# Aakash1312/Fluid-Simulation

Measured on AMD Instinct MI355X. Metric: simulated substeps/sec, higher is better.
Workload: dtype f64

## Files before the change

fluid-simulation_amd/_lib.py:

```python
import ctypes as C
import os

_HERE = os.path.dirname(os.path.abspath(__file__))
_SO = os.path.join(_HERE, "libfluid_hip.so")
if not os.path.exists(_SO):
    raise ImportError(
        f"{_SO} is missing: build it with `make -C {_HERE}` (hipcc --offload-arch=gfx950). "
        "This package has no CPU path.")
lib = C.CDLL(_SO)


class FluidError(RuntimeError):
    def __init__(self, code, msg):
        super().__init__(f"libfluid_hip error {code}: {msg}")
        self.code = code


class Params(C.Structure):
    _fields_ = [("n", C.c_int32), ("device", C.c_int32), ("dx", C.c_double), ("rho", C.c_double),
                ("gravity", C.c_double * 3), ("max_dt", C.c_double), ("outer_tol", C.c_double),
                ("update_frac", C.c_double), ("cg_tol", C.c_double), ("cg_max_iters", C.c_int32),
                ("max_outer_passes", C.c_int32), ("precision", C.c_int32), ("preconditioner", C.c_int32),
                ("flip_blend", C.c_double), ("solve_start", C.c_int32), ("mg_precision", C.c_int32),
                ("dist_solve", C.c_int32), ("pad_", C.c_int32)]
# ... 120 lines not shown
    ("fluid_download_particles", C.c_int, [_P, _P, _P]),
    ("fluid_num_particles", C.c_int64, [_P]),
    ("fluid_set_dt", C.c_int, [_P, C.c_double]),
    ("fluid_get_dt", C.c_int, [_P, C.POINTER(C.c_double)]),
    ("fluid_scene_water_cube_drop", C.c_int64, [C.c_int32, C.c_int32, C.c_uint64, _P]),
    ("fluid_scene_uniform_scatter", C.c_int64, [C.POINTER(C.c_int32), C.POINTER(C.c_int32), C.c_float, C.c_uint32, C.c_int32, _P]),
    ("fluid_step", C.c_int, [_P, C.POINTER(StepStats)]),
    ("fluid_p2g", C.c_int, [_P]),
    ("fluid_flags_index", C.c_int, [_P]),
    ("fluid_rhs_div", C.c_int, [_P, C.c_int]),
    ("fluid_solve", C.c_int, [_P]),
    ("fluid_vel_update", C.c_int, [_P]),
    ("fluid_pressure_pass", C.c_int, [_P, C.POINTER(C.c_double)]),
    ("fluid_flip_advect", C.c_int, [_P]),
    ("fluid_get_stats", C.c_int, [_P, C.POINTER(StepStats)]),
    ("fluid_download_field", C.c_int, [_P, C.c_int, _P, C.c_size_t]),
    ("fluid_upload_field", C.c_int, [_P, C.c_int, _P, C.c_size_t]),
    ("fluid_stencil_apply", C.c_int, [_P, C.c_int, C.c_int, C.POINTER(C.c_float)]),
    ("fluid_extrapolate", C.c_int, [_P, C.POINTER(C.c_int32)]),
    ("fluid_resample", C.c_int, [_P, C.c_int32, C.POINTER(C.c_int64)]),
    ("fluid_get_droplets", C.c_int, [_P, C.POINTER(C.c_int32), _P, C.c_int32]),
    ("fluid_add_particles", C.c_int, [_P, C.c_int64, _P, _P]),
    ("fluid_set_source", C.c_int, [_P, C.c_int32, C.POINTER(Source)]),
    ("fluid_set_sink", C.c_int, [_P, C.c_int32, C.POINTER(C.c_int32), C.POINTER(C.c_int32)]),
    ("fluid_get_source_stats", C.c_int, [_P, C.POINTER(C.c_int64), C.POINTER(C.c_int64), C.POINTER(C.c_int64), C.POINTER(C.c_int64)]),
    ("fluid_dist_set_source", C.c_int, [_P, C.c_int32, C.POINTER(Source)]),
    ("fluid_dist_set_sink", C.c_int, [_P, C.c_int32, C.POINTER(C.c_int32), C.POINTER(C.c_int32)]),
    ("fluid_dist_get_source_stats", C.c_int, [_P, C.POINTER(C.c_int64), C.POINTER(C.c_int64), C.POINTER(C.c_int64), C.POINTER(C.c_int64)]),
    ("fluid_dist_add_particles", C.c_int, [_P, C.c_int64, _P, _P, _P]),
    ("fluid_stencil_apply_hbm", C.c_int, [_P, C.c_int, C.c_int, C.c_int64, C.POINTER(C.c_int32), C.POINTER(C.c_float)]),
# ... 104 lines not shown
```

fluid-simulation_amd/csrc/fluid_api.hip:

```cpp
#include "sim.h"
#include <algorithm>

using namespace fl;

static thread_local std::string g_err;
int fluid_fail(int code, const std::string& msg)
{
    g_err = msg;
    return code;
}
#define fail fluid_fail

Box fl::clip_dilate(const Box& b, int d, const Grid& g)
{
    Box r;
    r.x0 = b.x0 - d < 0 ? 0 : b.x0 - d;
    r.y0 = b.y0 - d < 0 ? 0 : b.y0 - d;
    r.z0 = b.z0 - d < 0 ? 0 : b.z0 - d;
    r.x1 = b.x1 + d > g.nx - 1 ? g.nx - 1 : b.x1 + d;
    r.y1 = b.y1 + d > g.ny - 1 ? g.ny - 1 : b.y1 + d;
    r.z1 = b.z1 + d > g.nz - 1 ? g.nz - 1 : b.z1 + d;
    return r;
}

// ... 37 lines not shown
    }
}


static void free_particles(fluid_sim* s)
{
    for (Particles* p : {&s->pa, &s->pb}) {
        hipFree(p->px); hipFree(p->py); hipFree(p->pz); hipFree(p->vx); hipFree(p->vy); hipFree(p->vz); hipFree(p->pid);
        *p = Particles{};
    }
    hipFree(s->key); hipFree(s->slot); hipFree(s->order); hipFree(s->order2); hipFree(s->spid); hipFree(s->stage_pos); hipFree(s->stage_vel);
    s->order2 = nullptr; s->spid = nullptr; hipFree(s->pw);
    s->pw = nullptr;
    s->key = s->slot = s->order = nullptr;
    s->binned = false;
    s->stage_pos = s->stage_vel = nullptr;
    s->cap = 0;
}

int fl::alloc_particles(fluid_sim* s, long n)
{
    if (n <= s->cap) return FLUID_OK;
    n = (n + 1) & ~1L;
    free_particles(s);
    for (Particles* p : {&s->pa, &s->pb}) {
        HIPCHK(dalloc(&p->px, n)); HIPCHK(dalloc(&p->py, n)); HIPCHK(dalloc(&p->pz, n));
        HIPCHK(dalloc(&p->vx, n)); HIPCHK(dalloc(&p->vy, n)); HIPCHK(dalloc(&p->vz, n));
        HIPCHK(dalloc(&p->pid, n));
    }
    HIPCHK(dalloc(&s->key, n)); HIPCHK(dalloc(&s->slot, n)); HIPCHK(dalloc(&s->order, n)); HIPCHK(dalloc(&s->order2, n)); HIPCHK(dalloc(&s->spid, n));
    HIPCHK(dalloc(&s->stage_pos, 3 * n)); HIPCHK(dalloc(&s->stage_vel, 3 * n));
    HIPCHK(dalloc(&s->pw, 9 * n));
    HIPCHK(hipDeviceSynchronize());
    s->cap = n;
    return FLUID_OK;
}

int fl::grow_particles(fluid_sim* s, long need)
{
    if (need <= s->cap) return FLUID_OK;
    HIPCHK(hipStreamSynchronize(s->st));
    const long keep = s->p_off + s->np;
    Particles old = s->pa;
    s->pa = Particles{};
    const long ncap = ((need + need / 2) + 1) & ~1L;
    Particles nw{};
    HIPCHK(dalloc(&nw.px, ncap)); HIPCHK(dalloc(&nw.py, ncap)); HIPCHK(dalloc(&nw.pz, ncap));
    HIPCHK(dalloc(&nw.vx, ncap)); HIPCHK(dalloc(&nw.vy, ncap)); HIPCHK(dalloc(&nw.vz, ncap));
    HIPCHK(dalloc(&nw.pid, ncap));
    if (keep > 0) {
        HIPCHK(hipMemcpy(nw.px, old.px, keep * 8, hipMemcpyDeviceToDevice)); HIPCHK(hipMemcpy(nw.py, old.py, keep * 8, hipMemcpyDeviceToDevice));
        HIPCHK(hipMemcpy(nw.pz, old.pz, keep * 8, hipMemcpyDeviceToDevice)); HIPCHK(hipMemcpy(nw.vx, old.vx, keep * 8, hipMemcpyDeviceToDevice));
        HIPCHK(hipMemcpy(nw.vy, old.vy, keep * 8, hipMemcpyDeviceToDevice)); HIPCHK(hipMemcpy(nw.vz, old.vz, keep * 8, hipMemcpyDeviceToDevice));
        HIPCHK(hipMemcpy(nw.pid, old.pid, keep * 4, hipMemcpyDeviceToDevice));
    }
    hipFree(old.px); hipFree(old.py); hipFree(old.pz); hipFree(old.vx); hipFree(old.vy); hipFree(old.vz); hipFree(old.pid);
// ... 46 lines not shown
    if (s->st) hipStreamSynchronize(s->st);
    if (s->ds) dist_destroy(s);
    prof_resolve(s);
    free_particles(s);
    sources_free(s);
    output_free(s);
    render_free(s);
    mesh_free(s);
    sdf_free(s);
    void* ptrs[] = {s->solid, s->flags, s->container, s->rhs, s->diver, s->diver2, s->u, s->v, s->w, s->ub, s->vb, s->wb, s->dcx, s->dcy,
                    s->dcz, s->pressure, s->p_guess, s->p_guess2, s->p_q, s->indices, s->scan_sums, s->ipart, s->R, s->S[0], s->Q, s->X, s->mg_slab, s->mg_part, s->cntL, s->part_bb, s->part_rr,
                    s->part_rz[0], s->part_rz[1], s->part_pq, s->part_err, s->cell_count, s->cell_start, s->ss,
                    s->pcx, s->pcy, s->pcz, s->p2g_part, s->p2g_items, s->p2g_crowd, s->tl_flags, s->tl_mg, s->tl_sq, s->d_small, s->row_flags, s->row_pos, s->row_list, s->drop_n, s->drop_cells, s->drop_ctr, s->gal_slab};
    for (void* p : ptrs) if (p) hipFree(p);
    for (int i = 0; i < 2; ++i) if (s->ev_poll[i]) hipEventDestroy(s->ev_poll[i]);
    if (s->h_ss) hipHostFree(s->h_ss);
    if (s->h_small) hipHostFree(s->h_small);
    if (s->st) hipStreamDestroy(s->st);
    delete s;
    return FLUID_OK;
}

int fluid_create(const fluid_params_t* p, fluid_sim_t** out)
{
    if (!p || !out) return fail(FLUID_ERR_ARG, "null argument");
    Grid g;
    g.N = p->n;
    g.lo = -(p->n / 2);
    g.hi = g.lo + p->n - 1;
    g.nx = g.ny = g.nz = p->n;
// ... 23 lines not shown
    s->prm = *p;
    s->g = g;
    s->ncell = g.cells();
    s->dt = p->max_dt;
    s->mg_fp32 = p->mg_precision == FLUID_MG_FP32;
    s->warm = p->solve_start == FLUID_START_WARM;
    if (const char* e = getenv("FLUID_MG_CSWEEPS")) s->mg_csweeps = atoi(e);
    if (const char* e = getenv("FLUID_TILE_LISTS")) s->lists_force = atoi(e) != 0;
    if (const char* e = getenv("FLUID_P2G_FORM")) s->p2g_force = !strcmp(e, "rows") ? 1 : (!strcmp(e, "tiles") ? 2 : (!strcmp(e, "crowd") ? 3 : 0));
    if (const char* e = getenv("FLUID_MG_GALERKIN")) s->gal_mode = atoi(e);
    if (const char* e = getenv("FLUID_DROPLETS")) s->drops_on = atoi(e) != 0;
    if (const char* e = getenv("FLUID_ROW_SWEEPS")) s->row_sweeps = atoi(e) != 0;
    if (const char* e = getenv("FLUID_DROPLETS_MIN")) s->drop_min = atoi(e);
    if (const char* e = getenv("FLUID_ADVECT_BIN")) s->advect_bin = atoi(e) != 0;
    if (const char* e = getenv("FLUID_SOLVE_TAIL")) s->solve_tail = atoi(e) != 0;
    *out = nullptr;
    auto bail = [&](int rc) { fluid_destroy(s); return rc; };
#define A(expr) do { hipError_t e_ = (expr); if (e_ != hipSuccess) return bail(fail(FLUID_ERR_HIP, std::string(#expr) + ": " + hipGetErrorString(e_))); } while (0)
    A(hipStreamCreateWithFlags(&s->st, hipStreamNonBlocking));
    const size_t n = s->ncell;
    A(dalloc(&s->solid, n)); A(dalloc(&s->flags, n));
    A(dalloc(&s->container, n)); A(dalloc(&s->rhs, n)); A(dalloc(&s->diver, n)); A(dalloc(&s->diver2, n));
    A(dalloc(&s->u, n)); A(dalloc(&s->v, n)); A(dalloc(&s->w, n));
    A(dalloc(&s->ub, n)); A(dalloc(&s->vb, n)); A(dalloc(&s->wb, n));
    A(dalloc(&s->dcx, n)); A(dalloc(&s->dcy, n)); A(dalloc(&s->dcz, n));
    A(dalloc(&s->pressure, n));
    if (s->warm) {
        A(dalloc(&s->p_guess, n)); A(dalloc(&s->p_guess2, n));
        if (hipMemset(s->p_guess, 0, n * sizeof(double)) != hipSuccess || hipMemset(s->p_guess2, 0, n * sizeof(double)) != hipSuccess) return bail(FLUID_ERR_HIP);
        if (const char* e = getenv("FLUID_EXTRAPOLATE")) s->extrapolate = atoi(e) != 0;
// ... 8 lines not shown
    A(dalloc((char**)&s->R, ln * se)); A(dalloc((char**)&s->S[0], 2 * ln * se + 256));
    s->S[1] = (char*)s->S[0] + ln * se;
    A(dalloc((char**)&s->Q, ln * se)); A(dalloc((char**)&s->X, ln * se)); A(dalloc(&s->cntL, ln + 64));
    A(dalloc(&s->mg_part, ln / 256 + 64));
    A(dalloc(&s->part_bb, (size_t)MAX_PARTIALS)); A(dalloc(&s->part_rr, (size_t)MAX_PARTIALS));
    A(dalloc(&s->part_rz[0], (size_t)MAX_PARTIALS)); A(dalloc(&s->part_rz[1], (size_t)MAX_PARTIALS));
    A(dalloc(&s->part_pq, (size_t)MAX_PARTIALS)); A(dalloc(&s->part_err, (size_t)2 * MAX_PARTIALS));
    static_assert(sizeof(StepState) <= STATE_PS_OFF, "PcgState overlaps StepState");
    A(dalloc((char**)&s->ss, STATE_PS_OFF + sizeof(PcgState)));
    s->ps = (PcgState*)((char*)s->ss + STATE_PS_OFF);
    A(dalloc(&s->cell_count, n + 4)); A(dalloc(&s->cell_start, n + 4));
    A(dalloc(&s->d_small, (size_t)32));
    A(hipHostMalloc((void**)&s->h_small, 32 * sizeof(int)));
    A(hipEventCreateWithFlags(&s->ev_poll[0], hipEventDisableTiming));
    A(hipEventCreateWithFlags(&s->ev_poll[1], hipEventDisableTiming));
    A(hipHostMalloc((void**)&s->h_ss, STATE_PS_OFF + 2 * sizeof(PcgState)));
    s->h_ps = (PcgState*)((char*)s->h_ss + STATE_PS_OFF);
#undef A
    std::vector<uint8_t> sol(n, 0);
    const int N = p->n;
    for (int x = 0; x < g.nx; ++x)
        for (int y = 0; y < g.ny; ++y)
            for (int z = 0; z < g.nz; ++z) {
                const int X = x + g.ox, Y = y + g.oy, Z = z + g.oz;
                if (X < 2 || X > N - 3 || Y < 2 || Y > N - 3 || Z < 2 || Z > N - 3) sol[g.idx(x, y, z)] = 1;
            }
    hipError_t e = hipMemcpy(s->solid, sol.data(), n, hipMemcpyHostToDevice);
    if (e == hipSuccess) e = hipMemcpy(s->flags, sol.data(), n, hipMemcpyHostToDevice);
    if (e == hipSuccess) e = hipDeviceSynchronize();
    if (e != hipSuccess) return bail(fail(FLUID_ERR_HIP, std::string("solid upload: ") + hipGetErrorString(e)));
// ... 24 lines not shown
    HIPCHK(hipStreamSynchronize(s->st));
    HIPCHK(hipMemcpy(s->solid, sol.data(), s->ncell, hipMemcpyHostToDevice));
    HIPCHK(hipMemcpy(s->flags, sol.data(), s->ncell, hipMemcpyHostToDevice));
    s->have_p2g = s->have_flags = false;
    s->flags_valid = false;
    s->have_guess = false;
    return FLUID_OK;
}

int fluid_upload_particles(fluid_sim_t* s, int64_t n, const double* pos, const double* vel)
{
    if (!s || n < 0 || (n > 0 && !pos)) return fail(FLUID_ERR_ARG, "bad particle arguments");
    if (s->dist) return fail(FLUID_ERR_STATE, "decomposed run: use fluid_upload_particles_ids (global ids must be unique across ranks)");
    if (n > 0x7fffffffL) return fail(FLUID_ERR_ARG, "too many particles");
    HIPCHK(hipSetDevice(s->prm.device));
    int rc = alloc_particles(s, (long)n);
    if (rc) return rc;
    s->np = (long)n;
    s->p_off = 0;
    if (n > 0) {
        HIPCHK(hipMemcpyAsync(s->stage_pos, pos, 3 * n * sizeof(double), hipMemcpyHostToDevice, s->st));
        if (vel) HIPCHK(hipMemcpyAsync(s->stage_vel, vel, 3 * n * sizeof(double), hipMemcpyHostToDevice, s->st));
        launch_unpack_particles(s->st, s->np, s->stage_pos, vel ? s->stage_vel : nullptr, s->pa);
        HIPCHK(hipGetLastError());
        HIPCHK(hipStreamSynchronize(s->st));
    }
    s->sorted = s->have_p2g = s->have_flags = false;
    s->have_guess = false;
    s->sort_hint = false;
    s->binned = false;
    s->vel_ok = false;
    return FLUID_OK;
}

int fluid_download_particles(fluid_sim_t* s, double* pos, double* vel)
{
    if (!s || !pos || !vel) return fail(FLUID_ERR_ARG, "null argument");
    if (s->dist) return fail(FLUID_ERR_STATE, "decomposed run: use fluid_download_particles_ids");
    if (s->np == 0) return FLUID_OK;
    HIPCHK(hipSetDevice(s->prm.device));
    launch_pack_particles(s->st, s->np, s->pa.shifted(s->p_off), s->stage_pos, s->stage_vel);
    HIPCHK(hipGetLastError());
    HIPCHK(hipMemcpyAsync(pos, s->stage_pos, 3 * s->np * sizeof(double), hipMemcpyDeviceToHost, s->st));
    HIPCHK(hipMemcpyAsync(vel, s->stage_vel, 3 * s->np * sizeof(double), hipMemcpyDeviceToHost, s->st));
    HIPCHK(hipStreamSynchronize(s->st));
    return FLUID_OK;
}

int64_t fluid_num_particles(fluid_sim_t* s) { return s ? s->np : -1; }
int fluid_set_dt(fluid_sim_t* s, double dt)
{
    if (!s || !(dt > 0)) return fail(FLUID_ERR_ARG, "dt must be > 0");
    s->dt = dt;
    return FLUID_OK;
}
int fluid_get_dt(fluid_sim_t* s, double* dt)
// ... 31 lines not shown
                        cnt++;
                    }
                }
    return cnt;
}

}

int fl::read_ss(fluid_sim* s)
{
    HIPCHK(hipMemcpyAsync(s->h_ss, s->ss, sizeof(StepState), hipMemcpyDeviceToHost, s->st));
    HIPCHK(hipStreamSynchronize(s->st));
    return FLUID_OK;
}

int fl::clear_dirty(fluid_sim* s)
{
    if (box_empty(s->dirty)) return FLUID_OK;
    const ZeroList z = {{s->container, s->rhs, s->diver, s->diver2}, {s->u, s->v, s->w, s->ub, s->vb, s->wb, s->pressure}};
    launch_zero_fields(s->st, z, s->g, s->dirty, !s->dist && s->row_sweeps);
    HIPCHK(hipGetLastError());
    s->dirty = Box{0, 0, 0, -1, -1, -1};
    return FLUID_OK;
}

int fl::sort_pass(fluid_sim* s, int ax0, int ax1, int* h_tail)
{
    const Grid g = s->g;
    const long ncell = (long)s->ncell, n2 = g.sx();
    const long c0 = (long)ax0 * n2, c1 = (long)(ax1 + 1) * n2;
    launch_zero_step_state(s->st, s->ss, g.N);
    HIPCHK(hipMemsetAsync(s->cell_count + c0, 0, (c1 - c0) * sizeof(int), s->st));
    HIPCHK(hipMemsetAsync(s->cell_count + ncell, 0, 4 * sizeof(int), s->st));
    launch_bin_count(s->st, g, s->np, s->pa.shifted(s->p_off), s->key, s->slot, s->cell_count, s->ipart, s->ss);
    launch_exclusive_scan(s->st, s->cell_count + c0, s->cell_start + c0, c1 - c0, s->scan_sums, s->cell_start + c1);
    launch_sort_tail(s->st, s->cell_count, s->cell_start, c1, ncell);
    launch_bin_scatter(s->st, s->np, s->key, s->slot, s->cell_start, s->pa.shifted(s->p_off).pid, s->order, s->spid);
    launch_bin_rank(s->st, s->np, 0, s->key, s->cell_start, s->order, s->spid, s->order2);
    HIPCHK(hipGetLastError());
    if (h_tail) HIPCHK(hipMemcpyAsync(h_tail, s->cell_start + ncell, 3 * sizeof(int), hipMemcpyDeviceToHost, s->st));
    return read_ss(s);
}

static int sort_binned(fluid_sim* s)
{
    const Grid g = s->g;
    const long ncell = (long)s->ncell, n2 = g.sx();
    const long c0 = (long)s->bin_x0 * n2, c1 = (long)(s->bin_x1 + 1) * n2;
    launch_zero_step_state(s->st, s->ss, g.N);
    launch_exclusive_scan(s->st, s->cell_count + c0, s->cell_start + c0, c1 - c0, s->scan_sums, s->cell_start + c1);
    launch_sort_tail(s->st, s->cell_count, s->cell_start, c1, ncell);
    launch_bin_scatter(s->st, s->np, s->key, s->slot, s->cell_start, s->pa.shifted(s->p_off).pid, s->order, s->spid);
    launch_bin_rank(s->st, s->np, 0, s->key, s->cell_start, s->order, s->spid, s->order2);
    HIPCHK(hipGetLastError());
    StepState& h = *s->h_ss;
    for (int a = 0; a < 3; ++a) h.bbox_min[a] = s->bin_min[a], h.bbox_max[a] = s->bin_max[a];
    h.n_out = s->bin_n_out;
    h.max_cell = s->bin_max_cell;
    return FLUID_OK;
}

static int phase_sort(fluid_sim* s)
{
    const Grid g = s->g;
    int tok = prof_begin(s, FLUID_PROF_SORT, (double)s->np);
    int ax0 = 0, ax1 = g.nx - 1;
    const bool guess = s->sort_hint && !box_empty(s->Pb);
    if (guess) {
        ax0 = std::max(0, s->Pb.x0 - 3);
        ax1 = std::min(g.nx - 1, s->Pb.x1 + 3);
    }
    const bool binned = s->binned && guess && ax0 == s->bin_x0 && ax1 == s->bin_x1 && s->np > 0;
    s->binned = false;
    const auto missed = [&](const int* bmin, const int* bmax) {
        return guess && bmax[0] >= 0 && (bmin[0] < std::min(ax0 + 2, s->Pb.x0) || bmax[0] > std::max(ax1 - 2, s->Pb.x1));
    };
    int rc;
    if (binned && !missed(s->bin_min, s->bin_max)) {
        if ((rc = sort_binned(s))) return rc;
    } else {
        rc = binned ? FLUID_OK : sort_pass(s, ax0, ax1);
        if (rc) return rc;
        if (binned || missed(s->h_ss->bbox_min, s->h_ss->bbox_max)) {
            if ((rc = sort_pass(s, 0, g.nx - 1))) return rc;
        }
    }
    s->sort_hint = true;
    s->n_out = s->h_ss->n_out;
    s->max_cell = s->h_ss->max_cell;
    const StepState& h = *s->h_ss;
    if (h.bbox_max[0] < 0) {
        s->Pb = Box{0, 0, 0, -1, -1, -1};
    } else {
        s->Pb = Box{h.bbox_min[0], h.bbox_min[1], h.bbox_min[2], h.bbox_max[0], h.bbox_max[1], h.bbox_max[2]};
    }
    if (!box_empty(s->Pb)) {
        s->Rb = clip_dilate(s->Pb, 1, g);
        s->Sb = clip_dilate(s->Pb, 2, g);
    } else {
        s->Rb = s->Sb = s->Pb;
    }
    launch_reorder(s->st, s->np, s->order2, s->pa.shifted(s->p_off), s->pb, s->pw, s->cap);
    HIPCHK(hipGetLastError());
    std::swap(s->pa, s->pb);
    s->p_off = 0;
    prof_end(s, FLUID_PROF_SORT, tok);
    s->sorted = true;
    return FLUID_OK;
}

int fl::run_p2g(fluid_sim* s, const Box& box)
{
    const long ref_cells = s->p2g_ref_cells > 0 ? s->p2g_ref_cells : s->Rb.cells();
    const bool airy = s->last_num_active > 0 && (double)s->last_num_active < 0.3 * (double)ref_cells;
    const bool huge = (size_t)12 * sizeof(double) * (size_t)box.cells() > ((size_t)16 << 30);
    const bool piled = s->max_cell > P2G_PILED || airy;
    if (s->p2g_force ? s->p2g_force == 2 : huge) {
        s->stats.paths |= FLUID_PATH_P2G_TILES;
        launch_p2g_tiles(s->st, s->g, box, s->pa, s->pw, s->cap, s->cell_start, s->flags, s->container, s->u, s->v, s->w, s->ub, s->vb, s->wb);
        return FLUID_OK;
// ... 467 lines not shown
                    HIPCHK(hipStreamSynchronize(s->st));
                    hipFree(s->row_flags); hipFree(s->row_pos); hipFree(s->row_list);
                    s->row_flags = s->row_pos = s->row_list = nullptr;
                    const size_t cap = nr + nr / 4 + 1024;
                    HIPCHK(hipMalloc((void**)&s->row_flags, cap * sizeof(int)));
                    HIPCHK(hipMalloc((void**)&s->row_pos, cap * sizeof(int)));
                    HIPCHK(hipMalloc((void**)&s->row_list, cap * sizeof(int)));
                    s->row_cap = cap;
                }
                launch_row_list(s->st, s->L, s->cntL, s->row_flags, s->row_pos, s->row_list, s->scan_sums, &s->ss->n_rows);
            }
            built = true;
        }
        HIPCHK(hipGetLastError());
    }
    int rc = read_ss(s);
    if (rc) return rc;
    s->stats.num_active = s->h_ss->num_active;
    s->last_num_active = s->stats.num_active;
    s->lists_on = false;
    s->lists_hint = false;
    if (!box_empty(s->Rb)) {
        const bool airy = (double)s->stats.num_active < 0.45 * (double)s->L.cells() && s->L.cells() > (size_t)1500000;
        s->lists_hint = airy;
        s->n_tl_mg = s->h_ss->n_tl_mg; s->n_tl_sq = s->h_ss->n_tl_sq; s->n_rows = s->h_ss->n_rows;
        s->n_drop = drops ? std::min(s->h_ss->n_drop, DROP_CAP) : 0;
        if (drops) s->drop_last = s->n_drop;
        if (s->n_drop > 0) s->stats.paths |= FLUID_PATH_DROPLETS;
        s->lists_on = built && s->n_tl_mg > 0 && s->n_tl_sq > 0 && (s->lists_force == 1 || airy);
        if (s->lists_on) s->stats.paths |= FLUID_PATH_TILE_LISTS;
        const size_t lb = (s->L.cells() + 2 * (size_t)s->L.Lz) * solver_elem(s);
        HIPCHK(zero_search(s, lb));
        HIPCHK(hipGetLastError());
        if (use_mg(s)) {
            int rc2 = mg_setup(s);
            if (rc2) return rc2;
        }
    }
    s->have_flags = true;
    return FLUID_OK;
}

static int phase_rhs_div(fluid_sim* s, int which, const PcgState* gate)
{
    if (!s->have_flags) return fail(FLUID_ERR_STATE, "rhs_div before flags_index");
    if (box_empty(s->Rb)) return FLUID_OK;
    const double dt = s->dt;
    launch_rhs_div(s->st, s->g, s->Rb, s->flags, s->u, s->v, s->w, s->rhs, which ? s->diver2 : s->diver, s->prm.dx,
                   s->prm.gravity[0] * dt, s->prm.gravity[1] * dt, s->prm.gravity[2] * dt, !s->dist && s->row_sweeps, gate);
    HIPCHK(hipGetLastError());
    return FLUID_OK;
// ... 143 lines not shown
    prof_end(s, FLUID_PROF_G2P, tok);
    const bool bin = s->advect_bin && !s->dist && s->np > 0 && s->sorted && s->sort_hint && !box_empty(s->Pb);
    s->binned = false;
    if (bin) {
        const Grid g = s->g;
        s->bin_x0 = std::max(0, s->Pb.x0 - 3);
        s->bin_x1 = std::min(g.nx - 1, s->Pb.x1 + 3);
        const long n2 = g.sx(), c0 = (long)s->bin_x0 * n2, c1 = (long)(s->bin_x1 + 1) * n2;
        HIPCHK(hipMemsetAsync(s->cell_count + c0, 0, (c1 - c0) * sizeof(int), s->st));
        HIPCHK(hipMemsetAsync(s->cell_count + s->ncell, 0, 4 * sizeof(int), s->st));
        launch_advect_bin(s->st, g, s->np, s->pa.shifted(s->p_off), s->flags, s->prm.max_dt, s->prm.dx, s->ss, s->key, s->slot, s->cell_count, s->ipart);
    } else {
        launch_advect(s->st, s->g, s->np, s->pa.shifted(s->p_off), s->flags, s->prm.max_dt, s->prm.dx, s->ss);
    }
    HIPCHK(hipGetLastError());
    int rc = read_ss(s);
    if (rc) return rc;
    if (bin) {
        const StepState& h = *s->h_ss;
        for (int a = 0; a < 3; ++a) s->bin_min[a] = h.bbox_min[a], s->bin_max[a] = h.bbox_max[a];
        s->bin_n_out = h.n_out;
        s->bin_max_cell = h.max_cell;
        s->binned = true;
    }
    s->dt = s->h_ss->dt;
    double ms;
    memcpy(&ms, &s->h_ss->max_speed_bits, sizeof(double));
    s->stats.max_speed = ms;
    s->stats.dt_out = s->dt;
    s->sorted = false;
    s->have_p2g = false;
    s->vel_ok = true;
    return FLUID_OK;
}

extern "C" {

#define PHASE_GUARD(s)                                                                                        \
// ... 85 lines not shown
    HIPCHK(hipStreamSynchronize(s->st));
    if (n_parked) *n_parked = s->h_small[0];
    s->sorted = s->have_p2g = s->have_flags = false;
    s->sort_hint = false;
    s->binned = false;
    return FLUID_OK;
}

int fluid_get_stats(fluid_sim_t* s, fluid_step_stats_t* st)
{
    if (!s || !st) return fail(FLUID_ERR_ARG, "null argument");
    *st = s->stats;
    return FLUID_OK;
}


int fluid_step(fluid_sim_t* s, fluid_step_stats_t* stats)
{
    if (!s) return fail(FLUID_ERR_ARG, "null handle");
    int rc;
    if ((rc = output_auto_check(s))) return rc;
    if (s->dist) return dist_step(s, stats);
    if ((rc = phase_p2g(s))) return rc;
    if ((rc = phase_flags(s))) return rc;
    double error = NAN;
    do {
        if ((rc = phase_pressure_pass(s, &error))) return rc;
        if (s->prm.max_outer_passes > 0 && s->stats.outer_passes >= s->prm.max_outer_passes) break;
    } while (error > s->prm.outer_tol);
    if ((rc = phase_flip_advect(s))) return rc;
// ... 245 lines not shown
```

fluid-simulation_amd/csrc/fluid_dist.hip:

```cpp
#include "sim.h"
#include "dist_kernels.h"

using namespace fl;
#define fail fluid_fail
int cuts_from_hist(int n, const int64_t* hist, int P, int32_t* cuts);

#define COMMCHK(expr)                                                                              \
    do {                                                                                           \
        if ((expr) != 0) return fail(FLUID_ERR_HIP, std::string("comm callback failed: ") + #expr); \
    } while (0)

namespace {

constexpr int HALO_W = 4;

struct IBox {
    int lo[3], hi[3];
};
inline bool ib_empty(const IBox& b) { return b.hi[0] <= b.lo[0] || b.hi[1] <= b.lo[1] || b.hi[2] <= b.lo[2]; }
inline IBox ib_isect(const IBox& a, const IBox& b)
{
    IBox r;
    for (int k = 0; k < 3; ++k) { r.lo[k] = std::max(a.lo[k], b.lo[k]); r.hi[k] = std::min(a.hi[k], b.hi[k]); }
    if (ib_empty(r)) for (int k = 0; k < 3; ++k) { r.lo[k] = a.lo[k]; r.hi[k] = a.lo[k]; }
// ... 1688 lines not shown
    for (int a = 0; a < 3; ++a) {
        if (origin) origin[a] = o[a];
        if (dims) dims[a] = n[a];
        if (own_lo) own_lo[a] = s->ds ? s->ds->ob.lo[a] : 0;
        if (own_hi) own_hi[a] = s->ds ? s->ds->ob.hi[a] : g.N;
    }
    return FLUID_OK;
}

int fluid_upload_particles_ids(fluid_sim_t* s, int64_t n, const double* pos, const double* vel, const uint32_t* ids)
{
    if (!s || n < 0 || (n > 0 && (!pos || !ids))) return fail(FLUID_ERR_ARG, "bad particle arguments");
    HIPCHK(hipSetDevice(s->prm.device));
    long slack = 1L << 16;
    if (const char* e = getenv("FLUID_DIST_SLACK")) slack = std::max(16L, atol(e));
    int rc = alloc_particles(s, 2 * (long)n + slack);
    if (rc) return rc;
    DistState* d = s->ds;
    if (d && !d->mig_s) {
        d->mig_cap = (long)n / 2 + slack;
        HIPCHK(hipMalloc((void**)&d->mig_s, (size_t)d->mig_cap * 56));
        HIPCHK(hipMalloc((void**)&d->mig_r, (size_t)d->mig_cap * 56));
    }
    s->np = (long)n;
    s->p_off = 0;
    if (n > 0) {
        uint32_t* dids = (uint32_t*)s->order;
        HIPCHK(hipMemcpyAsync(s->stage_pos, pos, 3 * n * sizeof(double), hipMemcpyHostToDevice, s->st));
        if (vel) HIPCHK(hipMemcpyAsync(s->stage_vel, vel, 3 * n * sizeof(double), hipMemcpyHostToDevice, s->st));
        HIPCHK(hipMemcpyAsync(dids, ids, n * sizeof(uint32_t), hipMemcpyHostToDevice, s->st));
// ... 7 lines not shown
    if (d) {
        s->vel_ok = false;
        for (int64_t i = 0; i < n; ++i) d->max_id = std::max(d->max_id, (long long)ids[i]);
    }
    return FLUID_OK;
}

int64_t fluid_download_particles_ids(fluid_sim_t* s, double* pos, double* vel, uint32_t* ids)
{
    if (!s) return -1;
    if (hipSetDevice(s->prm.device) != hipSuccess) return -1;
    int* cursor = s->d_small;
    if (hipMemsetAsync(cursor, 0, sizeof(int), s->st) != hipSuccess) return -1;
    const bool fetch = pos && vel && ids;
    uint32_t* dids = (uint32_t*)s->order;
    launch_pack_live(s->st, s->np, s->pa.shifted(s->p_off), fetch ? s->stage_pos : nullptr, s->stage_vel, dids, cursor);
    int live = 0;
    if (hipMemcpyAsync(s->h_small, cursor, sizeof(int), hipMemcpyDeviceToHost, s->st) != hipSuccess) return -1;
    if (hipStreamSynchronize(s->st) != hipSuccess) return -1;
    live = s->h_small[0];
    if (!fetch || live == 0) return live;
    if (hipMemcpyAsync(pos, s->stage_pos, 3 * (size_t)live * sizeof(double), hipMemcpyDeviceToHost, s->st) != hipSuccess) return -1;
    if (hipMemcpyAsync(vel, s->stage_vel, 3 * (size_t)live * sizeof(double), hipMemcpyDeviceToHost, s->st) != hipSuccess) return -1;
    if (hipMemcpyAsync(ids, dids, (size_t)live * sizeof(uint32_t), hipMemcpyDeviceToHost, s->st) != hipSuccess) return -1;
    if (hipStreamSynchronize(s->st) != hipSuccess) return -1;
    return live;
}

int fluid_partition_blocks(int32_t n, int64_t np, const double* pos, const int32_t dims[3], int32_t* cuts_x, int32_t* cuts_y, int32_t* cuts_z)
{
    if (n < 8 || !dims || !cuts_x || !cuts_y || !cuts_z || (np > 0 && !pos)) return fail(FLUID_ERR_ARG, "bad argument");
// ... 125 lines not shown
```

fluid-simulation_amd/csrc/fluid_sdf.hip:

```cpp
#include "sim.h"

using namespace fl;
#define fail fluid_fail

constexpr size_t SDF_REC = FLUID_SDF_LEAF_BYTES;
struct SdfMeta {
    int wide = 0;
    int attr = 0;
    int n_leaves = 0;
    float bg = 0, R = 0, w = 0;
};
struct SdfState {
    long cell_cap = 0, part_cap = 0, leaf_cap = 0;
    int *cnt = nullptr, *start = nullptr, *cell_sums = nullptr;
    int* place = nullptr;
    double* spos = nullptr;
    float* tv = nullptr;
    float* tv2 = nullptr;
    bool filtered = false;
    int* ssrc = nullptr;
    uint32_t* tid = nullptr;
    float* tvel = nullptr;
    bool attr = false;
    float* tmin = nullptr;
// ... 111 lines not shown
    const float mn = std::fmax(0.0f, R - w);
    g.min2 = mn * mn;
    f->any = false;
    f->tv = nullptr, f->flags = nullptr;
    f->filt = filt, f->dilate = 4;
    f->attr = false, f->dist2 = false;
    f->tm = nullptr, f->tid = nullptr, f->tvel = nullptr, f->tmin = nullptr;
    return FLUID_OK;
}

int fl::sdf_front(fluid_sim* s, SdfFront* f)
{
    SdfState* o = s->sdf;
    SdfGeom& g = f->g;
    int rc;
    const Particles live = s->pa.shifted(s->p_off);
    int* box = o->h_small;
    if (s->np > 0) {
        launch_sdf_bbox(s->st, s->np, live, g.lo, g.hi, o->d_small, s->dist);
        HIPCHK(hipGetLastError());
        HIPCHK(hipMemcpyAsync(o->h_small, o->d_small, 6 * sizeof(int), hipMemcpyDeviceToHost, s->st));
        HIPCHK(hipStreamSynchronize(s->st));
    }
    if (s->np > 0 && box[3] >= box[0]) {
        for (int a = 0; a < 3; ++a)
            if (box[a] < g.lo || box[3 + a] > g.hi || box[3 + a] < box[a]) return fail(FLUID_ERR_HIP, "level set: particle box out of range");
        g.bx0 = box[0], g.by0 = box[1], g.bz0 = box[2];
        g.bnx = box[3] - box[0] + 1, g.bny = box[4] - box[1] + 1, g.bnz = box[5] - box[2] + 1;
        for (int a = 0; a < 3; ++a) {
            const int c0 = std::max(box[a] - f->dilate, g.lo), c1 = std::min(box[3 + a] + f->dilate, g.hi);
            g.l0[a] = (c0 - g.L0) >> 3;
// ... 214 lines not shown
```

fluid-simulation_amd/csrc/fluid_sources.hip:

```cpp
#include "sim.h"
#include <algorithm>

using namespace fl;
#define fail fluid_fail

const char* const fl::SRC_SINGLE = "these entry points are single-GPU only (they renumber the pids): a decomposed handle uses fluid_dist_set_source, fluid_dist_set_sink, fluid_dist_get_source_stats, fluid_dist_add_particles";
const char* const fl::SRC_DIST = "not a decomposed handle: a fluid_create handle uses the one-GPU entry points (fluid_set_source, fluid_set_sink, fluid_get_source_stats, fluid_add_particles)";

static bool index_box(const fluid_sim* s, const int32_t lo[3], const int32_t hi[3], Box& b)
{
    const int N = s->g.N;
    for (int a = 0; a < 3; ++a)
        if (lo[a] < 0 || hi[a] > N - 1 || lo[a] > hi[a]) return false;
    b = Box{lo[0], lo[1], lo[2], hi[0], hi[1], hi[2]};
    return true;
}

static int ensure_sums(fluid_sim* s)
{
    if (s->src_sums) return FLUID_OK;
    HIPCHK(hipMalloc((void**)&s->src_sums, ((size_t)INT32_MAX / 2048 + 16) * sizeof(int)));
    return FLUID_OK;
}

// ... 134 lines not shown
    std::swap(s->pa, s->pb);
    s->p_off = 0;
    s->np = n - r;
    *removed = r;
    return FLUID_OK;
}

int fl::sources_apply(fluid_sim* s)
{
    s->src_emit_last = s->src_rm_last = 0;
    bool any = false;
    for (int i = 0; i < FLUID_MAX_SINKS; ++i) any = any || s->sink_on[i];
    for (const auto& q : s->src) any = any || q.on;
    if (!any) return FLUID_OK;
    s->binned = false;
    const long t = s->n_steps;
    const int N = s->g.N;
    const OwnBox all{{0, 0, 0}, {N, N, N}, {0, 0, 0}, {0, 0, 0}};
    long removed = 0, emitted = 0;
    int rc = apply_sinks(s, &removed);
    if (rc) return rc;
    for (auto& q : s->src) {
        if (!q.on || t % q.src.every != 0) continue;
        const SrcDue u = source_due(s, q, t, all);
        long m = 0, mo = 0;
        if ((rc = source_count(s, u)) || (rc = source_plan(s, u, &m, &mo))) return rc;
        if (m == 0) continue;
        if ((rc = source_room(s, m))) return rc;
        const Particles p = s->pa.shifted(s->p_off + s->np);
        source_emit(s, u, p, (uint32_t)s->np);
// ... 62 lines not shown
    if (emitted_total) *emitted_total = s->src_emit_total;
    if (removed_total) *removed_total = s->src_rm_total;
    return FLUID_OK;
}

extern "C" {

int fluid_add_particles(fluid_sim_t* s, int64_t n, const double* pos, const double* vel)
{
    if (int rc = snap_guard(s, SRC_SINGLE)) return rc;
    if (n < 0 || (n > 0 && !pos)) return fail(FLUID_ERR_ARG, "bad particle arguments");
    if (!vel && !s->vel_ok) return fail(FLUID_ERR_STATE, "add_particles with vel == NULL needs the grid velocities of a completed step");
    if (s->np + (long)n > (long)INT32_MAX) return fail(FLUID_ERR_STATE, "more than INT32_MAX particles");
    if (n == 0) return FLUID_OK;
    HIPCHK(hipSetDevice(s->prm.device));
    int rc = grow_particles(s, s->p_off + s->np + (long)n);
    if (rc) return rc;
    HIPCHK(hipMemcpyAsync(s->stage_pos, pos, 3 * n * sizeof(double), hipMemcpyHostToDevice, s->st));
    if (vel) HIPCHK(hipMemcpyAsync(s->stage_vel, vel, 3 * n * sizeof(double), hipMemcpyHostToDevice, s->st));
    const Particles p = s->pa.shifted(s->p_off + s->np);
    launch_src_append(s->st, (long)n, s->stage_pos, vel ? s->stage_vel : nullptr, p, (uint32_t)s->np);
    if (!vel) launch_interp_from_grid(s->st, s->g, (long)n, p, s->u, s->v, s->w);
    HIPCHK(hipGetLastError());
    HIPCHK(hipStreamSynchronize(s->st));
    s->np += (long)n;
    s->sorted = s->have_p2g = s->have_flags = false;
    s->sort_hint = false;
    s->binned = false;
    return FLUID_OK;
}
// ... 21 lines not shown
```

fluid-simulation_amd/csrc/sim.h:

```cpp
#pragma once
#include "common.h"
#include "../../include/fluid_hip.h"

#include <cmath>
#include <cstdio>
#include <cstdlib>
#include <cstring>
#include <string>
#include <utility>
#include <vector>

int fluid_fail(int code, const std::string& msg);
#define HIPCHK(expr)                                                                                              \
    do {                                                                                                          \
        hipError_t e_ = (expr);                                                                                   \
        if (e_ != hipSuccess)                                                                                     \
            return fluid_fail(FLUID_ERR_HIP, std::string(#expr) + ": " + hipGetErrorString(e_) + " @" + std::to_string(__LINE__)); \
    } while (0)
#include "snap_ring.h"

using namespace fl;

struct ProfClass {
    long launches = 0, sampled = 0;
// ... 86 lines not shown
    long p2g_ref_cells = 0;
    long last_num_active = 0;
    StepState* ss = nullptr;
    StepState* h_ss = nullptr;
    Box Pb{0, 0, 0, -1, -1, -1}, Rb{0, 0, 0, -1, -1, -1}, Sb{0, 0, 0, -1, -1, -1};
    Box dirty{0, 0, 0, -1, -1, -1};
    int flag_x0 = 0, flag_x1 = -1;
    bool flags_valid = false;
    bool sorted = false, have_p2g = false, have_flags = false;
    long n_out = 0;
    bool sort_hint = false;
    bool advect_bin = true;
    bool binned = false;
    int bin_x0 = 0, bin_x1 = -1;
    int bin_min[3] = {0, 0, 0}, bin_max[3] = {-1, -1, -1}, bin_n_out = 0, bin_max_cell = 0;
    bool solve_tail = true;
    bool tail_ran = false;
    double dt = 0.1;
    fluid_step_stats_t stats{};
    static constexpr int MG_MAXL = 8;
    int mg_nl = 0, mg_tail = 0;
    long mg_last_iters_k[3] = {0, 0, 0};
    int pass_class() const { return stats.outer_passes < 2 ? stats.outer_passes : 2; }
    int mg_csweeps = 3;
    MLevel mgl[MG_MAXL];
    uint8_t *mg_typ[MG_MAXL] = {}, *mg_cnt[MG_MAXL] = {};
    int gal_mode = 1;
    int gal_it[2] = {-1, -1};
    int gal_since_probe = 0;
    bool gal_eligible = false;
// ... 61 lines not shown
inline int grid_leaves(const Grid& g) { return ((g.hi & ~7) - (g.lo & ~7)) / 8 + 1; }
inline int snap_guard(const fluid_sim* s, const char* why, bool want_dist = false)
{
    if (!s) return fluid_fail(FLUID_ERR_ARG, "null handle");
    return s->dist != want_dist ? fluid_fail(FLUID_ERR_STATE, why) : FLUID_OK;
}
constexpr const char* ATTR_SINGLE = "these surface attribute calls are single-GPU only: a decomposed handle gives a rank record with squared distances (fluid_dist_sdf_snapshot_attr) and the records merge on the host (fluid_sdf_attr_grids_merge)";
inline size_t solver_elem(const fluid_sim* s) { return s->prm.precision == FLUID_PRECISION_FP32 ? 4 : 8; }
inline bool use_mg(const fluid_sim* s) { return s->prm.preconditioner == FLUID_PRECOND_MG && s->prm.precision == FLUID_PRECISION_FP64; }

int prof_begin(fluid_sim* s, int k, double cells);
void prof_end(fluid_sim* s, int k, int tok);
int alloc_particles(fluid_sim* s, long n);
int grow_particles(fluid_sim* s, long need);
int read_ss(fluid_sim* s);
int sort_pass(fluid_sim* s, int ax0, int ax1, int* h_tail = nullptr);
int clear_dirty(fluid_sim* s);
int run_p2g(fluid_sim* s, const Box& box);
template <typename T>
Coef<T> make_coef(const fluid_sim* s);
MgCoef<double> mg_coef(const fluid_sim* s, int level);
hipError_t zero_search(fluid_sim* s, size_t lb);
int phase_flags(fluid_sim* s);
int phase_pressure_pass(fluid_sim* s, double* error);
int pic_fields(fluid_sim* s);
int fluid_create_window(const fluid_params_t* p, const Grid& g, fluid_sim_t** out);

int sources_apply(fluid_sim* s);
void sources_free(fluid_sim* s);
void sources_move(fluid_sim* from, fluid_sim* to);
// ... 61 lines not shown
```

fluid-simulation_amd/sim.py:

```python
import ctypes as C
import numpy as np

from ._lib import lib, check, FluidError, Params, StepStats, FIELD, Source, LeafGridC, SdfParams, SdfGridC, SdfFilter, MeshC, SdfAttrC, MeshAttrC, SdfAttrPartC, MeshExC, MESH, Camera, Shade, ImageC, RENDER

_FIELD_DTYPE = {
    FIELD.CONTAINER: (np.float32, 1), FIELD.WEIGHTS: (np.float32, 1), FIELD.OUTPUT: (np.float32, 1),
    FIELD.VEL: (np.float64, 3), FIELD.VEL_BEFORE: (np.float64, 3), FIELD.INDICES: (np.int32, 1),
    FIELD.RHS: (np.float32, 1), FIELD.DIVER: (np.float32, 1), FIELD.DIVER2: (np.float32, 1),
    FIELD.PRESSURE: (np.float64, 1), FIELD.SOLID: (np.uint8, 1), FIELD.FLAGS: (np.uint8, 1),
}


def grid_bounds(n):
    lo = -(n // 2)
    return lo, lo + n - 1


_VDB_COMPRESSION = {"zip": 3, "active_mask": 2}


def write_vdb(path, grids, compression="zip"):
    import ctypes as C
    if isinstance(grids, np.ndarray) and grids.ndim == 3:
        grids = [grids]
# ... 551 lines not shown
        check(lib.fluid_vel_update(self._h))

    def pressure_pass(self):
        e = C.c_double()
        check(lib.fluid_pressure_pass(self._h, C.byref(e)))
        return e.value

    def flip_advect(self):
        check(lib.fluid_flip_advect(self._h))

    def stats(self):
        st = StepStats()
        check(lib.fluid_get_stats(self._h, C.byref(st)))
        return st.as_dict()

    def _solver_dtype(self):
        return np.float64 if self.precision == "fp64" else np.float32

    def field(self, fid):
        if fid in (FIELD.SEARCH, FIELD.Q):
            dt, comps = self._solver_dtype(), 1
        else:
            dt, comps = _FIELD_DTYPE[fid]
        n = self.n
        arr = np.empty((comps, n, n, n) if comps > 1 else (n, n, n), dtype=dt)
        check(lib.fluid_download_field(self._h, fid, arr.ctypes.data_as(C.c_void_p), arr.nbytes))
        return arr

    def upload_field(self, fid, arr):
        if fid in (FIELD.SEARCH, FIELD.Q):
# ... 173 lines not shown
```

include/fluid_hip.h:

```cpp
#ifndef FLUID_HIP_H
#define FLUID_HIP_H

#include <stddef.h>
#include <stdint.h>

#ifdef __cplusplus
extern "C" {
#endif

typedef struct fluid_sim fluid_sim_t;

#define FLUID_OK 0
#define FLUID_ERR_ARG 1
#define FLUID_ERR_HIP 2
#define FLUID_ERR_STATE 3
#define FLUID_ERR_SOLVER 4
#define FLUID_ERR_PEER 5

#define FLUID_FIELD_CONTAINER 0
#define FLUID_FIELD_WEIGHTS 1
#define FLUID_FIELD_VEL 2
#define FLUID_FIELD_VEL_BEFORE 3
#define FLUID_FIELD_INDICES 4
#define FLUID_FIELD_RHS 5
// ... 82 lines not shown
int fluid_get_dt(fluid_sim_t* s, double* dt);
int64_t fluid_scene_water_cube_drop(int32_t n, int32_t ppc, uint64_t seed, double* pos);
int64_t fluid_scene_uniform_scatter(const int32_t lo[3], const int32_t hi[3], float points_per_volume, uint32_t seed,
                                    int32_t boundary, double* pos);

int fluid_step(fluid_sim_t* s, fluid_step_stats_t* stats);

int fluid_p2g(fluid_sim_t* s);
int fluid_flags_index(fluid_sim_t* s);
int fluid_rhs_div(fluid_sim_t* s, int which);
int fluid_solve(fluid_sim_t* s);
int fluid_vel_update(fluid_sim_t* s);
int fluid_pressure_pass(fluid_sim_t* s, double* error);
int fluid_flip_advect(fluid_sim_t* s);
int fluid_get_stats(fluid_sim_t* s, fluid_step_stats_t* stats);

int fluid_download_field(fluid_sim_t* s, int field, void* dst, size_t bytes);
int fluid_upload_field(fluid_sim_t* s, int field, const void* src, size_t bytes);

int fluid_extrapolate(fluid_sim_t* s, int32_t* n_layers);
int fluid_resample(fluid_sim_t* s, int32_t per_cell, int64_t* n_parked);

#define FLUID_MAX_SOURCES 8
#define FLUID_MAX_SINKS 8
#define FLUID_SOURCE_ADD 0
#define FLUID_SOURCE_FILL 1
#define FLUID_SOURCE_VEL_FIXED 0
#define FLUID_SOURCE_VEL_GRID 1
#define FLUID_PATH_SOURCES 512
typedef struct fluid_source {
// ... 228 lines not shown
```

Before: 159.2.

## Overlap step-state readback with next step's sort and multigrid setup

Replaces blocking step-state readbacks with an async copy plus event. While the host waits, it queues the next step's binned sort (scan, scatter, reorder) after advection, and the multigrid setup after flag indexing. Presorted particles are kept in the alternate buffer, and a presort_drop path restores them whenever particles are uploaded, grown, sourced or read, so later consumers see the live set. This is meant to hide host-device sync latency, at the cost of extra state and speculative work that must be thrown away when the bin bounds miss.

Measured after the change: 159.6 (median of 6 runs). No clear change (+0.3%).

```diff
diff --git a/fluid-simulation_amd/_lib.py b/fluid-simulation_amd/_lib.py
--- a/fluid-simulation_amd/_lib.py
+++ b/fluid-simulation_amd/_lib.py
@@ -158,6 +158,7 @@
     ("fluid_pressure_pass", C.c_int, [_P, C.POINTER(C.c_double)]),
     ("fluid_flip_advect", C.c_int, [_P]),
     ("fluid_get_stats", C.c_int, [_P, C.POINTER(StepStats)]),
+    ("fluid_step_ahead_info", C.c_int, [_P, C.POINTER(C.c_int64), C.POINTER(C.c_int64)]),
     ("fluid_download_field", C.c_int, [_P, C.c_int, _P, C.c_size_t]),
     ("fluid_upload_field", C.c_int, [_P, C.c_int, _P, C.c_size_t]),
     ("fluid_stencil_apply", C.c_int, [_P, C.c_int, C.c_int, C.POINTER(C.c_float)]),
diff --git a/fluid-simulation_amd/csrc/fluid_api.hip b/fluid-simulation_amd/csrc/fluid_api.hip
--- a/fluid-simulation_amd/csrc/fluid_api.hip
+++ b/fluid-simulation_amd/csrc/fluid_api.hip
@@ -75,6 +75,7 @@
     s->pw = nullptr;
     s->key = s->slot = s->order = nullptr;
     s->binned = false;
+    s->presorted = false;
     s->stage_pos = s->stage_vel = nullptr;
     s->cap = 0;
 }
@@ -101,6 +102,7 @@
 {
     if (need <= s->cap) return FLUID_OK;
     HIPCHK(hipStreamSynchronize(s->st));
+    presort_drop(s);
     const long keep = s->p_off + s->np;
     Particles old = s->pa;
     s->pa = Particles{};
@@ -177,6 +179,7 @@
                     s->pcx, s->pcy, s->pcz, s->p2g_part, s->p2g_items, s->p2g_crowd, s->tl_flags, s->tl_mg, s->tl_sq, s->d_small, s->row_flags, s->row_pos, s->row_list, s->drop_n, s->drop_cells, s->drop_ctr, s->gal_slab};
     for (void* p : ptrs) if (p) hipFree(p);
     for (int i = 0; i < 2; ++i) if (s->ev_poll[i]) hipEventDestroy(s->ev_poll[i]);
+    if (s->ev_ss) hipEventDestroy(s->ev_ss);
     if (s->h_ss) hipHostFree(s->h_ss);
     if (s->h_small) hipHostFree(s->h_small);
     if (s->st) hipStreamDestroy(s->st);
@@ -230,6 +233,7 @@
     if (const char* e = getenv("FLUID_DROPLETS_MIN")) s->drop_min = atoi(e);
     if (const char* e = getenv("FLUID_ADVECT_BIN")) s->advect_bin = atoi(e) != 0;
     if (const char* e = getenv("FLUID_SOLVE_TAIL")) s->solve_tail = atoi(e) != 0;
+    if (const char* e = getenv("FLUID_STEP_AHEAD")) { const int v = atoi(e); s->ahead_sort = v == 1 || v == 2; s->ahead_setup = v == 1 || v == 3; }
     *out = nullptr;
     auto bail = [&](int rc) { fluid_destroy(s); return rc; };
 #define A(expr) do { hipError_t e_ = (expr); if (e_ != hipSuccess) return bail(fail(FLUID_ERR_HIP, std::string(#expr) + ": " + hipGetErrorString(e_))); } while (0)
@@ -268,6 +272,7 @@
     A(hipHostMalloc((void**)&s->h_small, 32 * sizeof(int)));
     A(hipEventCreateWithFlags(&s->ev_poll[0], hipEventDisableTiming));
     A(hipEventCreateWithFlags(&s->ev_poll[1], hipEventDisableTiming));
+    A(hipEventCreateWithFlags(&s->ev_ss, hipEventDisableTiming));
     A(hipHostMalloc((void**)&s->h_ss, STATE_PS_OFF + 2 * sizeof(PcgState)));
     s->h_ps = (PcgState*)((char*)s->h_ss + STATE_PS_OFF);
 #undef A
@@ -322,6 +327,7 @@
     if (s->dist) return fail(FLUID_ERR_STATE, "decomposed run: use fluid_upload_particles_ids (global ids must be unique across ranks)");
     if (n > 0x7fffffffL) return fail(FLUID_ERR_ARG, "too many particles");
     HIPCHK(hipSetDevice(s->prm.device));
+    presort_drop(s);
     int rc = alloc_particles(s, (long)n);
     if (rc) return rc;
     s->np = (long)n;
@@ -347,7 +353,7 @@
     if (s->dist) return fail(FLUID_ERR_STATE, "decomposed run: use fluid_download_particles_ids");
     if (s->np == 0) return FLUID_OK;
     HIPCHK(hipSetDevice(s->prm.device));
-    launch_pack_particles(s->st, s->np, s->pa.shifted(s->p_off), s->stage_pos, s->stage_vel);
+    launch_pack_particles(s->st, s->np, live_particles(s), s->stage_pos, s->stage_vel);
     HIPCHK(hipGetLastError());
     HIPCHK(hipMemcpyAsync(pos, s->stage_pos, 3 * s->np * sizeof(double), hipMemcpyDeviceToHost, s->st));
     HIPCHK(hipMemcpyAsync(vel, s->stage_vel, 3 * s->np * sizeof(double), hipMemcpyDeviceToHost, s->st));
@@ -409,6 +415,26 @@
     return FLUID_OK;
 }
 
+int fl::read_ss_begin(fluid_sim* s)
+{
+    HIPCHK(hipMemcpyAsync(s->h_ss, s->ss, sizeof(StepState), hipMemcpyDeviceToHost, s->st));
+    HIPCHK(hipEventRecord(s->ev_ss, s->st));
+    return FLUID_OK;
+}
+int fl::read_ss_end(fluid_sim* s)
+{
+    HIPCHK(hipEventSynchronize(s->ev_ss));
+    return FLUID_OK;
+}
+
+void fl::presort_drop(fluid_sim* s)
+{
+    if (!s->presorted) return;
+    std::swap(s->pa, s->pb);
+    s->p_off = s->pre_off;
+    s->presorted = false;
+}
+
 int fl::clear_dirty(fluid_sim* s)
 {
     if (box_empty(s->dirty)) return FLUID_OK;
@@ -437,7 +463,7 @@
     return read_ss(s);
 }
 
-static int sort_binned(fluid_sim* s)
+static int sort_binned_scan(fluid_sim* s)
 {
     const Grid g = s->g;
     const long ncell = (long)s->ncell, n2 = g.sx();
@@ -445,20 +471,35 @@
     launch_zero_step_state(s->st, s->ss, g.N);
     launch_exclusive_scan(s->st, s->cell_count + c0, s->cell_start + c0, c1 - c0, s->scan_sums, s->cell_start + c1);
     launch_sort_tail(s->st, s->cell_count, s->cell_start, c1, ncell);
+    HIPCHK(hipGetLastError());
+    return FLUID_OK;
+}
+static int sort_binned_place(fluid_sim* s)
+{
     launch_bin_scatter(s->st, s->np, s->key, s->slot, s->cell_start, s->pa.shifted(s->p_off).pid, s->order, s->spid);
     launch_bin_rank(s->st, s->np, 0, s->key, s->cell_start, s->order, s->spid, s->order2);
     HIPCHK(hipGetLastError());
+    return FLUID_OK;
+}
+static void sort_binned_host(fluid_sim* s)
+{
     StepState& h = *s->h_ss;
     for (int a = 0; a < 3; ++a) h.bbox_min[a] = s->bin_min[a], h.bbox_max[a] = s->bin_max[a];
     h.n_out = s->bin_n_out;
     h.max_cell = s->bin_max_cell;
+}
+static int sort_reorder(fluid_sim* s)
+{
+    launch_reorder(s->st, s->np, s->order2, s->pa.shifted(s->p_off), s->pb, s->pw, s->cap);
+    HIPCHK(hipGetLastError());
+    std::swap(s->pa, s->pb);
+    s->p_off = 0;
     return FLUID_OK;
 }
 
 static int phase_sort(fluid_sim* s)
 {
     const Grid g = s->g;
-    int tok = prof_begin(s, FLUID_PROF_SORT, (double)s->np);
     int ax0 = 0, ax1 = g.nx - 1;
     const bool guess = s->sort_hint && !box_empty(s->Pb);
     if (guess) {
@@ -471,8 +512,13 @@
         return guess && bmax[0] >= 0 && (bmin[0] < std::min(ax0 + 2, s->Pb.x0) || bmax[0] > std::max(ax1 - 2, s->Pb.x1));
     };
     int rc;
+    const bool ahead = s->presorted && binned && !missed(s->bin_min, s->bin_max);
+    if (!ahead) presort_drop(s);
+    s->presorted = false;
+    const int tok = ahead ? -1 : prof_begin(s, FLUID_PROF_SORT, (double)s->np);
     if (binned && !missed(s->bin_min, s->bin_max)) {
-        if ((rc = sort_binned(s))) return rc;
+        if (!ahead && ((rc = sort_binned_scan(s)) || (rc = sort_binned_place(s)))) return rc;
+        sort_binned_host(s);
     } else {
         rc = binned ? FLUID_OK : sort_pass(s, ax0, ax1);
         if (rc) return rc;
@@ -495,10 +541,7 @@
     } else {
         s->Rb = s->Sb = s->Pb;
     }
-    launch_reorder(s->st, s->np, s->order2, s->pa.shifted(s->p_off), s->pb, s->pw, s->cap);
-    HIPCHK(hipGetLastError());
-    std::swap(s->pa, s->pb);
-    s->p_off = 0;
+    if (!ahead && (rc = sort_reorder(s))) return rc;
     prof_end(s, FLUID_PROF_SORT, tok);
     s->sorted = true;
     return FLUID_OK;
@@ -996,7 +1039,20 @@
         }
         HIPCHK(hipGetLastError());
     }
-    int rc = read_ss(s);
+    const size_t lb = box_empty(s->Rb) ? 0 : (s->L.cells() + 2 * (size_t)s->L.Lz) * solver_elem(s);
+    const bool early = s->ahead_setup && !s->dist && !box_empty(s->Rb) && !built && use_mg(s);
+    int rc;
+    if (early) {
+        if ((rc = read_ss_begin(s))) return rc;
+        s->lists_on = false;
+        HIPCHK(zero_search(s, lb));
+        const int rc2 = mg_setup(s);
+        if ((rc = read_ss_end(s))) return rc;
+        if (rc2) return rc2;
+        s->early_setups++;
+    } else {
+        rc = read_ss(s);
+    }
     if (rc) return rc;
     s->stats.num_active = s->h_ss->num_active;
     s->last_num_active = s->stats.num_active;
@@ -1011,12 +1067,13 @@
         if (s->n_drop > 0) s->stats.paths |= FLUID_PATH_DROPLETS;
         s->lists_on = built && s->n_tl_mg > 0 && s->n_tl_sq > 0 && (s->lists_force == 1 || airy);
         if (s->lists_on) s->stats.paths |= FLUID_PATH_TILE_LISTS;
-        const size_t lb = (s->L.cells() + 2 * (size_t)s->L.Lz) * solver_elem(s);
-        HIPCHK(zero_search(s, lb));
-        HIPCHK(hipGetLastError());
-        if (use_mg(s)) {
-            int rc2 = mg_setup(s);
-            if (rc2) return rc2;
+        if (!early) {
+            HIPCHK(zero_search(s, lb));
+            HIPCHK(hipGetLastError());
+            if (use_mg(s)) {
+                int rc2 = mg_setup(s);
+                if (rc2) return rc2;
+            }
         }
     }
     s->have_flags = true;
@@ -1190,7 +1247,18 @@
         launch_advect(s->st, s->g, s->np, s->pa.shifted(s->p_off), s->flags, s->prm.max_dt, s->prm.dx, s->ss);
     }
     HIPCHK(hipGetLastError());
-    int rc = read_ss(s);
+    bool ahead = bin && s->ahead_sort && !(s->out_every > 0 && s->n_steps % s->out_every == 0);
+    for (int i = 0; i < FLUID_MAX_SINKS; ++i) ahead = ahead && !s->sink_on[i];
+    for (const auto& q : s->src) ahead = ahead && !q.on;
+    int rc, tok2 = -1;
+    if (ahead) {
+        if ((rc = read_ss_begin(s))) return rc;
+        tok2 = prof_begin(s, FLUID_PROF_SORT, (double)s->np);
+        if ((rc = sort_binned_scan(s))) return rc;
+        rc = read_ss_end(s);
+    } else {
+        rc = read_ss(s);
+    }
     if (rc) return rc;
     if (bin) {
         const StepState& h = *s->h_ss;
@@ -1198,6 +1266,16 @@
         s->bin_n_out = h.n_out;
         s->bin_max_cell = h.max_cell;
         s->binned = true;
+    }
+    if (ahead) {
+        const bool missed = s->bin_max[0] >= 0 && (s->bin_min[0] < std::min(s->bin_x0 + 2, s->Pb.x0) || s->bin_max[0] > std::max(s->bin_x1 - 2, s->Pb.x1));
+        if (!missed) {
+            s->pre_off = s->p_off;
+            if ((rc = sort_binned_place(s)) || (rc = sort_reorder(s))) return rc;
+            s->presorted = true;
+            s->presorted_steps++;
+        }
+        prof_end(s, FLUID_PROF_SORT, tok2);
     }
     s->dt = s->h_ss->dt;
     double ms;
@@ -1313,6 +1391,13 @@
     return FLUID_OK;
 }
 
+int fluid_step_ahead_info(fluid_sim_t* s, int64_t* presorted_steps, int64_t* early_setups)
+{
+    if (!s) return fail(FLUID_ERR_ARG, "null handle");
+    if (presorted_steps) *presorted_steps = s->presorted_steps;
+    if (early_setups) *early_setups = s->early_setups;
+    return FLUID_OK;
+}
 
 int fluid_step(fluid_sim_t* s, fluid_step_stats_t* stats)
 {
diff --git a/fluid-simulation_amd/csrc/fluid_dist.hip b/fluid-simulation_amd/csrc/fluid_dist.hip
--- a/fluid-simulation_amd/csrc/fluid_dist.hip
+++ b/fluid-simulation_amd/csrc/fluid_dist.hip
@@ -1726,6 +1726,7 @@
     HIPCHK(hipSetDevice(s->prm.device));
     long slack = 1L << 16;
     if (const char* e = getenv("FLUID_DIST_SLACK")) slack = std::max(16L, atol(e));
+    presort_drop(s);
     int rc = alloc_particles(s, 2 * (long)n + slack);
     if (rc) return rc;
     DistState* d = s->ds;
@@ -1763,7 +1764,7 @@
     if (hipMemsetAsync(cursor, 0, sizeof(int), s->st) != hipSuccess) return -1;
     const bool fetch = pos && vel && ids;
     uint32_t* dids = (uint32_t*)s->order;
-    launch_pack_live(s->st, s->np, s->pa.shifted(s->p_off), fetch ? s->stage_pos : nullptr, s->stage_vel, dids, cursor);
+    launch_pack_live(s->st, s->np, live_particles(s), fetch ? s->stage_pos : nullptr, s->stage_vel, dids, cursor);
     int live = 0;
     if (hipMemcpyAsync(s->h_small, cursor, sizeof(int), hipMemcpyDeviceToHost, s->st) != hipSuccess) return -1;
     if (hipStreamSynchronize(s->st) != hipSuccess) return -1;
diff --git a/fluid-simulation_amd/csrc/fluid_sdf.hip b/fluid-simulation_amd/csrc/fluid_sdf.hip
--- a/fluid-simulation_amd/csrc/fluid_sdf.hip
+++ b/fluid-simulation_amd/csrc/fluid_sdf.hip
@@ -149,7 +149,7 @@
     SdfState* o = s->sdf;
     SdfGeom& g = f->g;
     int rc;
-    const Particles live = s->pa.shifted(s->p_off);
+    const Particles live = live_particles(s);
     int* box = o->h_small;
     if (s->np > 0) {
         launch_sdf_bbox(s->st, s->np, live, g.lo, g.hi, o->d_small, s->dist);
diff --git a/fluid-simulation_amd/csrc/fluid_sources.hip b/fluid-simulation_amd/csrc/fluid_sources.hip
--- a/fluid-simulation_amd/csrc/fluid_sources.hip
+++ b/fluid-simulation_amd/csrc/fluid_sources.hip
@@ -172,6 +172,7 @@
     for (const auto& q : s->src) any = any || q.on;
     if (!any) return FLUID_OK;
     s->binned = false;
+    presort_drop(s);
     const long t = s->n_steps;
     const int N = s->g.N;
     const OwnBox all{{0, 0, 0}, {N, N, N}, {0, 0, 0}, {0, 0, 0}};
@@ -264,6 +265,7 @@
     if (s->np + (long)n > (long)INT32_MAX) return fail(FLUID_ERR_STATE, "more than INT32_MAX particles");
     if (n == 0) return FLUID_OK;
     HIPCHK(hipSetDevice(s->prm.device));
+    presort_drop(s);
     int rc = grow_particles(s, s->p_off + s->np + (long)n);
     if (rc) return rc;
     HIPCHK(hipMemcpyAsync(s->stage_pos, pos, 3 * n * sizeof(double), hipMemcpyHostToDevice, s->st));
diff --git a/fluid-simulation_amd/csrc/sim.h b/fluid-simulation_amd/csrc/sim.h
--- a/fluid-simulation_amd/csrc/sim.h
+++ b/fluid-simulation_amd/csrc/sim.h
@@ -124,6 +124,11 @@
     bool binned = false;
     int bin_x0 = 0, bin_x1 = -1;
     int bin_min[3] = {0, 0, 0}, bin_max[3] = {-1, -1, -1}, bin_n_out = 0, bin_max_cell = 0;
+    bool ahead_sort = true, ahead_setup = true;
+    hipEvent_t ev_ss = nullptr;
+    bool presorted = false;
+    long pre_off = 0;
+    long presorted_steps = 0, early_setups = 0;
     bool solve_tail = true;
     bool tail_ran = false;
     double dt = 0.1;
@@ -215,6 +220,10 @@
 int alloc_particles(fluid_sim* s, long n);
 int grow_particles(fluid_sim* s, long need);
 int read_ss(fluid_sim* s);
+int read_ss_begin(fluid_sim* s);
+int read_ss_end(fluid_sim* s);
+void presort_drop(fluid_sim* s);
+inline Particles live_particles(const fluid_sim* s) { return s->presorted ? s->pb.shifted(s->pre_off) : s->pa.shifted(s->p_off); }
 int sort_pass(fluid_sim* s, int ax0, int ax1, int* h_tail = nullptr);
 int clear_dirty(fluid_sim* s);
 int run_p2g(fluid_sim* s, const Box& box);
diff --git a/fluid-simulation_amd/sim.py b/fluid-simulation_amd/sim.py
--- a/fluid-simulation_amd/sim.py
+++ b/fluid-simulation_amd/sim.py
@@ -589,6 +589,11 @@
         check(lib.fluid_get_stats(self._h, C.byref(st)))
         return st.as_dict()
 
+    def step_ahead_info(self):
+        a, b = C.c_int64(), C.c_int64()
+        check(lib.fluid_step_ahead_info(self._h, C.byref(a), C.byref(b)))
+        return {"presorted_steps": a.value, "early_setups": b.value}
+
     def _solver_dtype(self):
         return np.float64 if self.precision == "fp64" else np.float32
 
diff --git a/include/fluid_hip.h b/include/fluid_hip.h
--- a/include/fluid_hip.h
+++ b/include/fluid_hip.h
@@ -120,6 +120,7 @@
 int fluid_pressure_pass(fluid_sim_t* s, double* error);
 int fluid_flip_advect(fluid_sim_t* s);
 int fluid_get_stats(fluid_sim_t* s, fluid_step_stats_t* stats);
+int fluid_step_ahead_info(fluid_sim_t* s, int64_t* presorted_steps, int64_t* early_setups);
 
 int fluid_download_field(fluid_sim_t* s, int field, void* dst, size_t bytes);
 int fluid_upload_field(fluid_sim_t* s, int field, const void* src, size_t bytes);
```
